# hkust-vgd/nerfstyle

Hardware: AMD Instinct MI355X
Metric: train Mrays/sec (higher is better)
Workload: dtype f16

## Files before the change

### nerfstyle_amd/csrc/table_scatter.hip

```cpp
#include "field_common.h"
#include "table_scatter.h"


__device__ __forceinline__ bool seq_nonzero(const float4 &v) {
    return ((__float_as_uint(v.x) | __float_as_uint(v.y) | __float_as_uint(v.z) | __float_as_uint(v.w)) << 1) != 0u;
}

__device__ __forceinline__ uint32_t lat_row(const NsrLevel &lv, uint32_t x, uint32_t y, uint32_t z) {
    if (lv.use_hash) {
        const uint32_t index = x ^ (y * 2654435761u) ^ (z * 805459861u);
        if ((lv.size & (lv.size - 1u)) == 0u) return index & (lv.size - 1u);
        const uint32_t t = __umulhi(lv.magic, index);
        const uint32_t q = (t + ((index - t) >> lv.sh1)) >> lv.sh2;
        return index - q * lv.size;
    }
    return __umul24(x, lv.mul[0]) + __umul24(y, lv.mul[1]) + __umul24(z, lv.mul[2]);
}

struct LatGeom {
    uint16_t base[16];
    uint8_t S[16];
    uint8_t shift[16];
};
constexpr int TS_THREADS = 256;
constexpr int LAT_MAX_SLOTS = (int)(((65536 - 16 * sizeof(NsrLevel)) / (TS_THREADS / 64) - 256) / 16 / 64 * 64);
constexpr int LAT_KEY_BITS = 10;
constexpr uint32_t LAT_NONE = 0xFFFFFFFFu;
struct LatState {
    uint32_t b0, b1, b2;
};

static uint32_t lat_corners(uint32_t res, uint32_t shift) {
    const uint64_t span = (uint64_t)res << shift, blocks = 1u << LAT_KEY_BITS;
    const uint32_t cells = (span % blocks == 0) ? (uint32_t)(span / blocks) : (uint32_t)(span / blocks) + 2u;
    return cells + 1u;
}

static bool lat_geometry(const NsrLevel *lv, LatGeom &g) {
    uint32_t total = 0;
    for (int l = 0; l < 16; l++) {
        const uint32_t res = lv[l].resolution;
        uint32_t shift = 0, S = lat_corners(res, 0);
        while (shift < (uint32_t)LAT_KEY_BITS && lat_corners(res, shift + 1) <= (S > 3u ? S : 3u)) shift++;
        S = lat_corners(res, shift) > S ? lat_corners(res, shift) : S;
        if (S < 2u || S > 6u) return false;
        g.S[l] = (uint8_t)S;
        g.shift[l] = (uint8_t)shift;
        g.base[l] = (uint16_t)total;
        total += S * S * S;
    }
    return ((total + 63u) & ~63u) <= (uint32_t)LAT_MAX_SLOTS;
}

template <int S>
__device__ __forceinline__ void lat_flush_level(float4 *__restrict__ lat4, uint32_t *__restrict__ rows, uint32_t b0, uint32_t b1, uint32_t b2,
                                                const NsrLevel &lv, float *__restrict__ gt, int lane, bool td, bool tc) {
    constexpr int NC = S * S * S;
    const int t = lane >> 2, i = lane & 3;
    const bool on = (i < 2) ? td : tc;
    const float *lf = reinterpret_cast<const float *>(lat4);
#pragma unroll
    for (int k0 = 0; k0 < NC; k0 += 64) {
        const int k = k0 + lane;
        float4 v = make_float4(0.f, 0.f, 0.f, 0.f);
        if (k < NC) v = lat4[k];
        const bool nz = seq_nonzero(v);
        const unsigned long long m = __ballot(nz);
        if (m == 0ull) continue;
        if (nz) {
            constexpr uint32_t MZ = (65536u + S * S - 1u) / (S * S), MY = (65536u + S - 1u) / S;
            const uint32_t z = __umul24((uint32_t)k, MZ) >> 16, r = (uint32_t)k - __umul24(z, (uint32_t)(S * S));
            const uint32_t y = __umul24(r, MY) >> 16, x = r - __umul24(y, (uint32_t)S);
            rows[lane] = lv.offset + lat_row(lv, b0 + x, b1 + y, b2 + z);
        }
        __builtin_amdgcn_wave_barrier();
#pragma unroll
        for (int q = 0; q < 4; q++) {
            if (k0 + 16 * q >= NC) break;
            if (((m >> (16 * q)) & 0xFFFFull) == 0ull) continue;
            const bool rec = (m >> (16 * q + t)) & 1ull;
            if (rec) {
                const float val = lf[(k0 + 16 * q + t) * 4 + i];
                const uint32_t row = rows[16 * q + t];
                if (on) atomicAdd(gt + (size_t)row * 4 + i, val);
            }
        }
        __builtin_amdgcn_wave_barrier();
        if (nz) lat4[k] = make_float4(0.f, 0.f, 0.f, 0.f);
    }
}

__device__ __forceinline__ void lat_flush_dispatch(float4 *__restrict__ lat, int fl, const LatState &st,
                                                   const NsrLevel *__restrict__ lds_lv, float *__restrict__ gt, int lane, bool td, bool tc) {
    const uint32_t o0 = (uint32_t)__builtin_amdgcn_readlane((int)st.b0, fl * 4);
    if (o0 == LAT_NONE) return;
    const uint32_t o1 = (uint32_t)__builtin_amdgcn_readlane((int)st.b1, fl * 4);
    const uint32_t o2 = (uint32_t)__builtin_amdgcn_readlane((int)st.b2, fl * 4);
    const NsrLevel flv = lds_lv[fl];
    float4 *lf = lat + (flv.pad_ >> 8);
    uint32_t *rows = reinterpret_cast<uint32_t *>(lat) - 64;
    switch (flv.pad_ & 0xFu) {
    case 3: lat_flush_level<3>(lf, rows, o0, o1, o2, flv, gt, lane, td, tc); break;
    case 4: lat_flush_level<4>(lf, rows, o0, o1, o2, flv, gt, lane, td, tc); break;
    case 5: lat_flush_level<5>(lf, rows, o0, o1, o2, flv, gt, lane, td, tc); break;
    default: lat_flush_level<6>(lf, rows, o0, o1, o2, flv, gt, lane, td, tc); break;
    }
}


struct TableScatterArgs {
    const float *xyzs;
    const uint32_t *perm;
    const int32_t *m_dev;
    uint32_t M;
    const float4 *gin;
    float *grad_tables;
    float bmin[3], bsize[3];
    int td, tc;
    uint32_t lat_slots;
    NsrLevel lv[16];
};

constexpr int TS_RING = 8;
static size_t ts_wave_bytes(uint32_t lat_slots) { return 256 + (size_t)lat_slots * 16; }

__global__ void __launch_bounds__(TS_THREADS)
k_table_scatter(TableScatterArgs a) {
    extern __shared__ __attribute__((aligned(16))) char smem[];
    NsrLevel *lds_lv = reinterpret_cast<NsrLevel *>(smem);
    if (threadIdx.x < 16) lds_lv[threadIdx.x] = a.lv[threadIdx.x];
    const int lane = threadIdx.x & 63, wave = threadIdx.x >> 6;
    char *base = smem + 16 * sizeof(NsrLevel) + (size_t)wave * (256 + (size_t)a.lat_slots * 16);
    float4 *lat = reinterpret_cast<float4 *>(base + 256);
    for (uint32_t k = lane; k < a.lat_slots; k += 64) lat[k] = make_float4(0.f, 0.f, 0.f, 0.f);
    __syncthreads();

    const uint32_t Mc = a.m_dev ? min((uint32_t)max(a.m_dev[0], 0), a.M) : a.M;
    if (Mc == 0) return;
    const uint32_t ntiles = (Mc + 15) / 16;
    const uint32_t nwaves = gridDim.x * (TS_THREADS / 64), gw = blockIdx.x * (TS_THREADS / 64) + wave;
    const uint32_t per = (ntiles + nwaves - 1) / nwaves;
    const uint32_t w_begin = min(gw * per, ntiles), w_end = min(w_begin + per, ntiles);
    if (w_begin >= w_end) return;
    const int s = lane & 15;
    const int l = lane >> 2, py = lane & 1, pz = (lane >> 1) & 1;
    const NsrLevel lv = lds_lv[l];
    const uint32_t S = lv.pad_ & 0xFu, ashift = (lv.pad_ >> 4) & 0xFu;
    float4 *const mylat = lat + (lv.pad_ >> 8) + ((uint32_t)pz * S + (uint32_t)py) * S;
    const bool td = a.td != 0, tc = a.tc != 0;
    float *const gt = a.grad_tables;
    const float kq = (float)(1 << LAT_KEY_BITS), rk = 1.0f / kq;
    LatState st;
    st.b0 = st.b1 = st.b2 = LAT_NONE;
    uint32_t cur_key = LAT_NONE;
    float bf0 = 0.f, bf1 = 0.f, bf2 = 0.f;
    const float lscale = (float)lv.resolution;
    const float lcmax = (float)(lv.resolution - 1u);
    const float Sf = (float)S, Sm2 = (float)(S - 2u);
    const float sy = py ? 1.0f : -1.0f, oy = py ? 0.0f : 1.0f, sz = pz ? 1.0f : -1.0f, oz = pz ? 0.0f : 1.0f;

    auto fetch_idx = [&](uint32_t tile) -> uint32_t { return a.perm[min(tile * 16 + (uint32_t)s, Mc - 1u)]; };
    uint32_t idx = fetch_idx(w_begin);
    uint32_t idx_next = w_begin + 1 < w_end ? fetch_idx(w_begin + 1) : idx;
    float x0 = a.xyzs[(size_t)idx * 3], x1 = a.xyzs[(size_t)idx * 3 + 1], x2 = a.xyzs[(size_t)idx * 3 + 2];
    auto ts_gin = [&](uint32_t v, int ln) { return a.gin[(size_t)(uint32_t)__builtin_amdgcn_readlane((int)v, ln) * 16 + l]; };
    float4 gq[TS_RING];
#pragma unroll
    for (int i = 0; i < TS_RING; i++) gq[i] = ts_gin(idx, i);

    for (uint32_t tile = w_begin; tile < w_end; tile++) {
        float nx0 = x0, nx1 = x1, nx2 = x2;
        uint32_t idx_nn = idx_next;
        if (tile + 1 < w_end) {
            nx0 = a.xyzs[(size_t)idx_next * 3]; nx1 = a.xyzs[(size_t)idx_next * 3 + 1]; nx2 = a.xyzs[(size_t)idx_next * 3 + 2];
            if (tile + 2 < w_end) idx_nn = fetch_idx(tile + 2);
        }
        const bool valid = tile * 16 + (uint32_t)s < Mc;
        const float u0 = field_unit(x0, a.bmin[0], a.bsize[0]), u1 = field_unit(x1, a.bmin[1], a.bsize[1]),
                    u2 = field_unit(x2, a.bmin[2], a.bsize[2]);
        const bool live = valid && (u0 >= 0 && u0 <= 1 && u1 >= 0 && u1 <= 1 && u2 >= 0 && u2 <= 1);
        const uint32_t live16 = (uint32_t)(__ballot(live) & 0xFFFFull);
        const uint32_t q0 = (uint32_t)fminf(fmaxf(u0 * kq, 0.0f), kq - 1.0f), q1 = (uint32_t)fminf(fmaxf(u1 * kq, 0.0f), kq - 1.0f),
                       q2 = (uint32_t)fminf(fmaxf(u2 * kq, 0.0f), kq - 1.0f);
        const uint32_t bkey = q0 | (q1 << LAT_KEY_BITS) | (q2 << (2 * LAT_KEY_BITS));
        const uint32_t bkey_e = live ? bkey : LAT_NONE;
        const uint32_t bkey_l = (uint32_t)__builtin_amdgcn_update_dpp((int)cur_key, (int)bkey_e, 0x111, 0xF, 0xF, false);
        const uint32_t chg16 = (uint32_t)(__ballot(bkey_e != bkey_l) & 0xFFFFull);
#pragma unroll 1
        for (int part = 0; part < 16 / TS_RING; part++) {
            const bool wrap = part == 16 / TS_RING - 1;
            const uint32_t src = wrap ? idx_next : idx;
            const int src_lane0 = wrap ? 0 : (part + 1) * TS_RING;
#pragma unroll
            for (int ri = 0; ri < TS_RING; ri++) {
                const int step = part * TS_RING + ri;
                const float4 gr = gq[ri];
                if ((live16 >> step) & 1u) {
                    uint32_t key = cur_key;
                    if ((chg16 >> step) & 1u) key = (uint32_t)__builtin_amdgcn_readlane((int)bkey, step);
                    if (key != cur_key) {
                        cur_key = key;
                        const uint32_t kq0 = key & ((1u << LAT_KEY_BITS) - 1u), kq1 = (key >> LAT_KEY_BITS) & ((1u << LAT_KEY_BITS) - 1u),
                                       kq2 = key >> (2 * LAT_KEY_BITS);
                        const float o0 = (float)((kq0 >> ashift) << ashift) * rk, o1 = (float)((kq1 >> ashift) << ashift) * rk,
                                    o2 = (float)((kq2 >> ashift) << ashift) * rk;
                        float ff;
                        uint32_t n0, n1, n2;
                        nsr_grid_locate(o0, lv.resolution, 1, ff, n0);
                        nsr_grid_locate(o1, lv.resolution, 1, ff, n1);
                        nsr_grid_locate(o2, lv.resolution, 1, ff, n2);
                        const bool chg = (n0 != st.b0) | (n1 != st.b1) | (n2 != st.b2);
                        unsigned long long mm = __ballot(chg);
                        while (mm) {
                            const int fl = (int)(__builtin_ctzll(mm) >> 2);
                            mm &= ~(0xFull << (fl * 4));
                            lat_flush_dispatch(lat, fl, st, lds_lv, gt, lane, td, tc);
                        }
                        if (chg) { st.b0 = n0; st.b1 = n1; st.b2 = n2; bf0 = (float)n0; bf1 = (float)n1; bf2 = (float)n2; }
                    }
                    const float su0 = __builtin_bit_cast(float, __builtin_amdgcn_readlane(__builtin_bit_cast(int, u0), step));
                    const float su1 = __builtin_bit_cast(float, __builtin_amdgcn_readlane(__builtin_bit_cast(int, u1), step));
                    const float su2 = __builtin_bit_cast(float, __builtin_amdgcn_readlane(__builtin_bit_cast(int, u2), step));
                    float f0, f1, f2, cf0, cf1, cf2;
                    {
#pragma clang fp contract(off)
                        const float p0 = su0 * lscale, p1 = su1 * lscale, p2 = su2 * lscale;
                        cf0 = fminf(floorf(p0), lcmax); cf1 = fminf(floorf(p1), lcmax); cf2 = fminf(floorf(p2), lcmax);
                        f0 = p0 - cf0; f1 = p1 - cf1; f2 = p2 - cf2;
                    }
                    const float d0 = cf0 - bf0, d1 = cf1 - bf1, d2 = cf2 - bf2;
                    const float r0 = fminf(d0, Sm2), r1 = fminf(d1, Sm2), r2 = fminf(d2, Sm2);
                    const float wyz = fmaf(f1, sy, oy) * fmaf(f2, sz, oz);
                    float wB = f0 * wyz, wA = wyz - wB;
                    if (fmaxf(d0, fmaxf(d1, d2)) > Sm2) {
                        const uint32_t c0 = (uint32_t)cf0, c1 = (uint32_t)cf1, c2 = (uint32_t)cf2;
                        const uint32_t rowA = lv.offset + lat_row(lv, c0, c1 + (uint32_t)py, c2 + (uint32_t)pz);
                        const uint32_t rowB = lv.offset + lat_row(lv, c0 + 1u, c1 + (uint32_t)py, c2 + (uint32_t)pz);
                        const float ga[4] = {gr.x, gr.y, gr.z, gr.w};
#pragma unroll
                        for (int i = 0; i < 4; i++) {
                            if ((i < 2 ? td : tc) && ga[i] != 0.0f) {
                                atomicAdd(gt + (size_t)rowA * 4 + i, wA * ga[i]);
                                atomicAdd(gt + (size_t)rowB * 4 + i, wB * ga[i]);
                            }
                        }
                        wA = 0.0f;
                        wB = 0.0f;
                    }
                    float4 *const slot = mylat + (uint32_t)fmaf(fmaf(r2, Sf, r1), Sf, r0);
                    float4 va = slot[0], vb = slot[1];
                    va.x = fmaf(wA, gr.x, va.x); va.y = fmaf(wA, gr.y, va.y); va.z = fmaf(wA, gr.z, va.z); va.w = fmaf(wA, gr.w, va.w);
                    vb.x = fmaf(wB, gr.x, vb.x); vb.y = fmaf(wB, gr.y, vb.y); vb.z = fmaf(wB, gr.z, vb.z); vb.w = fmaf(wB, gr.w, vb.w);
                    slot[0] = va;
                    slot[1] = vb;
                }
                asm volatile("" ::: "memory");
                gq[ri] = ts_gin(src, src_lane0 + ri);
            }
        }
        x0 = nx0; x1 = nx1; x2 = nx2;
        idx = idx_next;
        idx_next = idx_nn;
    }
    __builtin_amdgcn_wave_barrier();
#pragma unroll 1
    for (int fl = 0; fl < 16; fl++) lat_flush_dispatch(lat, fl, st, lds_lv, gt, lane, td, tc);
}

bool nsr_table_scatter_supported(const NsrLevel *lv) {
    LatGeom g;
    return lat_geometry(lv, g);
}

int nsr_table_scatter_launch(const NsrLevel *levels, const float *bmin, const float *bsize, const float *xyzs, const uint32_t *perm,
                             const int32_t *m_dev, uint32_t M, const void *gin, float *grad_tables, int td, int tc, hipStream_t s) {
    TableScatterArgs a;
    LatGeom g;
    if (!lat_geometry(levels, g)) return NSR_ERR_UNSUPPORTED;
    uint32_t total = 0;
    for (int l = 0; l < 16; l++) {
        a.lv[l] = levels[l];
        a.lv[l].pad_ = (uint32_t)g.S[l] | ((uint32_t)g.shift[l] << 4) | ((uint32_t)g.base[l] << 8);
        total = g.base[l] + (uint32_t)g.S[l] * g.S[l] * g.S[l];
    }
    a.lat_slots = (total + 63u) & ~63u;
    a.xyzs = xyzs; a.perm = perm; a.m_dev = m_dev; a.M = M; a.gin = (const float4 *)gin; a.grad_tables = grad_tables;
    for (int i = 0; i < 3; i++) { a.bmin[i] = bmin[i]; a.bsize[i] = bsize[i]; }
    a.td = td; a.tc = tc;
    const size_t lds = 16 * sizeof(NsrLevel) + (TS_THREADS / 64) * ts_wave_bytes(a.lat_slots);
    static bool attr_set[64] = {};
    int dev = 0;
    (void)hipGetDevice(&dev);
    if (!attr_set[dev & 63]) {
        if (hipFuncSetAttribute(reinterpret_cast<const void *>(&k_table_scatter), hipFuncAttributeMaxDynamicSharedMemorySize, 65536) != hipSuccess)
            return NSR_ERR_LAUNCH;
        attr_set[dev & 63] = true;
    }
    if (lds > 65536) return NSR_ERR_UNSUPPORTED;
    uint32_t nblocks = 256u * 16u;
    const uint32_t ntiles = (M + 15) / 16;
    if (nblocks > (ntiles + 3) / 4) nblocks = (ntiles + 3) / 4;
    if (nblocks == 0) nblocks = 1;
    hipLaunchKernelGGL(k_table_scatter, dim3(nblocks), dim3(TS_THREADS), lds, s, a);
    return nsr_launch_status();
}
```

Baseline: 22.18.

## Carry overlapping lattice cells across window shifts along x instead of flushing

When a level's local lattice window moves only along x by less than its width, the flush writes out only the cells that leave the window. It shifts the surviving nonzero cells down in LDS so they keep accumulating, which cuts global atomicAdds for cells that would be re-touched. The flush loop is reorganised into row-aligned groups of 16 lanes (RS = floor(16/S)*S) so the shift stays inside one row. This adds extra barriers and LDS writes, wastes lanes when S does not divide 16, and drops the unroll of the flush loop.

```diff
diff --git a/nerfstyle_amd/csrc/table_scatter.hip b/nerfstyle_amd/csrc/table_scatter.hip
--- a/nerfstyle_amd/csrc/table_scatter.hip
+++ b/nerfstyle_amd/csrc/table_scatter.hip
@@ -54,56 +54,63 @@
 
 template <int S>
 __device__ __forceinline__ void lat_flush_level(float4 *__restrict__ lat4, uint32_t *__restrict__ rows, uint32_t b0, uint32_t b1, uint32_t b2,
-                                                const NsrLevel &lv, float *__restrict__ gt, int lane, bool td, bool tc) {
+                                                const NsrLevel &lv, float *__restrict__ gt, int lane, bool td, bool tc, uint32_t xl) {
     constexpr int NC = S * S * S;
+    constexpr int RS = (16 / S) * S;
     const int t = lane >> 2, i = lane & 3;
+    const int g = lane >> 4, j = lane & 15;
     const bool on = (i < 2) ? td : tc;
     const float *lf = reinterpret_cast<const float *>(lat4);
-#pragma unroll
-    for (int k0 = 0; k0 < NC; k0 += 64) {
-        const int k = k0 + lane;
+#pragma unroll 1
+    for (int k0 = 0; k0 < NC; k0 += 4 * RS) {
+        const int k = k0 + g * RS + j;
         float4 v = make_float4(0.f, 0.f, 0.f, 0.f);
-        if (k < NC) v = lat4[k];
+        if (j < RS && k < NC) v = lat4[k];
         const bool nz = seq_nonzero(v);
-        const unsigned long long m = __ballot(nz);
-        if (m == 0ull) continue;
+        if (__ballot(nz) == 0ull) continue;
+        bool out = false;
         if (nz) {
             constexpr uint32_t MZ = (65536u + S * S - 1u) / (S * S), MY = (65536u + S - 1u) / S;
             const uint32_t z = __umul24((uint32_t)k, MZ) >> 16, r = (uint32_t)k - __umul24(z, (uint32_t)(S * S));
             const uint32_t y = __umul24(r, MY) >> 16, x = r - __umul24(y, (uint32_t)S);
-            rows[lane] = lv.offset + lat_row(lv, b0 + x, b1 + y, b2 + z);
+            out = x < xl;
+            if (out) rows[lane] = lv.offset + lat_row(lv, b0 + x, b1 + y, b2 + z);
         }
+        const unsigned long long m = __ballot(out);
         __builtin_amdgcn_wave_barrier();
 #pragma unroll
         for (int q = 0; q < 4; q++) {
-            if (k0 + 16 * q >= NC) break;
+            if (k0 + RS * q >= NC) break;
             if (((m >> (16 * q)) & 0xFFFFull) == 0ull) continue;
             const bool rec = (m >> (16 * q + t)) & 1ull;
             if (rec) {
-                const float val = lf[(k0 + 16 * q + t) * 4 + i];
+                const float val = lf[(k0 + RS * q + t) * 4 + i];
                 const uint32_t row = rows[16 * q + t];
                 if (on) atomicAdd(gt + (size_t)row * 4 + i, val);
             }
         }
         __builtin_amdgcn_wave_barrier();
         if (nz) lat4[k] = make_float4(0.f, 0.f, 0.f, 0.f);
-    }
-}
-
-__device__ __forceinline__ void lat_flush_dispatch(float4 *__restrict__ lat, int fl, const LatState &st,
+        __builtin_amdgcn_wave_barrier();
+        if (nz && !out) lat4[k - (int)xl] = v;
+    }
+}
+
+__device__ __forceinline__ void lat_flush_dispatch(float4 *__restrict__ lat, int fl, const LatState &st, uint32_t xl_lane,
                                                    const NsrLevel *__restrict__ lds_lv, float *__restrict__ gt, int lane, bool td, bool tc) {
     const uint32_t o0 = (uint32_t)__builtin_amdgcn_readlane((int)st.b0, fl * 4);
     if (o0 == LAT_NONE) return;
     const uint32_t o1 = (uint32_t)__builtin_amdgcn_readlane((int)st.b1, fl * 4);
     const uint32_t o2 = (uint32_t)__builtin_amdgcn_readlane((int)st.b2, fl * 4);
+    const uint32_t xl = (uint32_t)__builtin_amdgcn_readlane((int)xl_lane, fl * 4);
     const NsrLevel flv = lds_lv[fl];
     float4 *lf = lat + (flv.pad_ >> 8);
     uint32_t *rows = reinterpret_cast<uint32_t *>(lat) - 64;
     switch (flv.pad_ & 0xFu) {
-    case 3: lat_flush_level<3>(lf, rows, o0, o1, o2, flv, gt, lane, td, tc); break;
-    case 4: lat_flush_level<4>(lf, rows, o0, o1, o2, flv, gt, lane, td, tc); break;
-    case 5: lat_flush_level<5>(lf, rows, o0, o1, o2, flv, gt, lane, td, tc); break;
-    default: lat_flush_level<6>(lf, rows, o0, o1, o2, flv, gt, lane, td, tc); break;
+    case 3: lat_flush_level<3>(lf, rows, o0, o1, o2, flv, gt, lane, td, tc, xl); break;
+    case 4: lat_flush_level<4>(lf, rows, o0, o1, o2, flv, gt, lane, td, tc, xl); break;
+    case 5: lat_flush_level<5>(lf, rows, o0, o1, o2, flv, gt, lane, td, tc, xl); break;
+    default: lat_flush_level<6>(lf, rows, o0, o1, o2, flv, gt, lane, td, tc, xl); break;
     }
 }
 
@@ -210,11 +217,14 @@
                         nsr_grid_locate(o1, lv.resolution, 1, ff, n1);
                         nsr_grid_locate(o2, lv.resolution, 1, ff, n2);
                         const bool chg = (n0 != st.b0) | (n1 != st.b1) | (n2 != st.b2);
+                        const uint32_t dx = n0 - st.b0;
+                        const bool carry = (st.b0 != LAT_NONE) & (n1 == st.b1) & (n2 == st.b2) & (dx - 1u < S - 1u);
+                        const uint32_t xl = carry ? dx : S;
                         unsigned long long mm = __ballot(chg);
                         while (mm) {
                             const int fl = (int)(__builtin_ctzll(mm) >> 2);
                             mm &= ~(0xFull << (fl * 4));
-                            lat_flush_dispatch(lat, fl, st, lds_lv, gt, lane, td, tc);
+                            lat_flush_dispatch(lat, fl, st, xl, lds_lv, gt, lane, td, tc);
                         }
                         if (chg) { st.b0 = n0; st.b1 = n1; st.b2 = n2; bf0 = (float)n0; bf1 = (float)n1; bf2 = (float)n2; }
                     }
@@ -264,7 +274,7 @@
     }
     __builtin_amdgcn_wave_barrier();
 #pragma unroll 1
-    for (int fl = 0; fl < 16; fl++) lat_flush_dispatch(lat, fl, st, lds_lv, gt, lane, td, tc);
+    for (int fl = 0; fl < 16; fl++) lat_flush_dispatch(lat, fl, st, S, lds_lv, gt, lane, td, tc);
 }
 
 bool nsr_table_scatter_supported(const NsrLevel *lv) {
```

After: 22.73, median of 6. 1.02x the previous value.
